# yoseph007/PQA2

Measured on AMD Instinct MI355X. Metric: VMAF frames/sec (vif+adm+motion2 -> SVM), device-resident synthetic YUV pairs, higher is better.
Workload: dtype f32; 1 GPU; 2160p 3840x2160 8-bit, vmaf_4k_v0.6.1, 300 frames/GPU; frames_per_gpu=300, frames_total=300, batch=97, frames_per_launch=75, clips_pipelined=True, parallelism=frame-shard x1, 1-frame motion halo, all-gather of records + of scores

## Files before the change

include/pqa_vmaf.h:

```cpp
#ifndef PQA_VMAF_H
#define PQA_VMAF_H

#include <stddef.h>
#include <stdint.h>

#if defined(__GNUC__)
#define PQA_API __attribute__((visibility("default")))
#else
#define PQA_API
#endif

#ifdef __cplusplus
extern "C" {
#endif

typedef enum pqa_status {
  PQA_OK = 0,
  PQA_EINVAL = -1,
  PQA_EDEVICE = -2,
  PQA_ENOMEM = -3,
  PQA_ECANCELLED = -4,
  PQA_ESTATE = -5
} pqa_status;

// ... 335 lines not shown
  uint32_t width, height;
} pqa_edge_spec;
PQA_API int pqa_edge_profiles(pqa_ctx* ctx, const pqa_edge_spec* spec, const void* const* ref_frames, int64_t ref_row_stride,
                              const void* const* dis_frames, int64_t dis_row_stride, int32_t n_frames, uint64_t* out);
PQA_API int pqa_edge_profiles_device(pqa_ctx* ctx, const pqa_edge_spec* spec, const void* ref, int64_t ref_row_pitch,
                                     int64_t ref_frame_pitch, const void* dis, int64_t dis_row_pitch, int64_t dis_frame_pitch,
                                     int32_t n_frames, uint64_t* out);
PQA_API int pqa_edge_sums(void);

PQA_API int pqa_colour_sums(void);
PQA_API int pqa_colour_moments_device(pqa_ctx* ctx, const pqa_device_clip* ref, const pqa_device_clip* dis, int32_t n_frames,
                                      uint32_t lo, uint32_t hi, uint64_t* out);
PQA_API int pqa_colour_moments(pqa_ctx* ctx, const void* const* ref_frames, const int64_t ref_strides[3],
                               const void* const* dis_frames, const int64_t dis_strides[3], int32_t n_frames, uint32_t lo,
                               uint32_t hi, uint64_t* out);

PQA_API int pqa_colour_apply_device(pqa_ctx* ctx, const int32_t m[12], const pqa_device_clip* src, const pqa_device_clip* dst,
                                    int32_t n_frames);
PQA_API int pqa_colour_apply(pqa_ctx* ctx, const int32_t m[12], const void* const* src_frames, const int64_t src_strides[3],
                             void* const* dst_frames, const int64_t dst_strides[3], int32_t n_frames);

enum { PQA_GRAY_LUMA = 0, PQA_GRAY_BT601_FULL = 1 };
PQA_API int pqa_set_luma_gray(pqa_ctx* ctx, uint32_t mode);

enum { PQA_PROF_KERNELS = 17 };
PQA_API int pqa_profile_enable(pqa_ctx* ctx, int on);
PQA_API int pqa_profile_read(pqa_ctx* ctx, int kernel_id, double* total_ms, uint64_t* launches, uint64_t* frames);
PQA_API const char* pqa_profile_kernel_name(int kernel_id);

PQA_API int pqa_debug_vif_march_table(uint16_t* out, int32_t capacity_halfwords);

PQA_API int pqa_debug_vif_march_shape(uint32_t width, uint32_t height, int32_t* out6);

PQA_API int pqa_debug_ciede2000(const double* lab_pairs, int32_t n, double* de_out);

enum { PQA_CAMBI_PARAM_INTS = 22 };
PQA_API int pqa_debug_cambi_params(uint32_t w, uint32_t h, uint32_t bit_depth, int32_t* out, int32_t cap);

PQA_API int pqa_debug_cambi_cmap(const void* luma, int64_t row_pitch_bytes, uint32_t w, uint32_t h, uint32_t bit_depth,
                                 float* cmap, int64_t cap, double* score);

PQA_API int pqa_debug_psnr_hvs_dct8x8(const int32_t* in, int32_t* out, int32_t n);

enum { PQA_PSNR_HVS_TABLE_FLOATS = 384 };
PQA_API int pqa_debug_psnr_hvs_tables(float* out, int32_t cap);

PQA_API int pqa_debug_psnr_hvs_plane(const void* ref, const void* dis, int64_t row_pitch_bytes, uint32_t w, uint32_t h,
                                     uint32_t bit_depth, uint32_t plane_kind, float* block_err, double* mse);

PQA_API int pqa_debug_xpsnr_blocks(const void* ref, const void* ref_m1, const void* ref_m2, const void* dis,
                                   int64_t row_pitch_bytes, uint32_t w, uint32_t h, uint32_t bit_depth, int32_t hfr,
                                   uint64_t* out, double* wsse);

PQA_API int pqa_debug_siti_plane(const void* cur, const void* prev, int64_t row_pitch_bytes, uint32_t w, uint32_t h,
                                 uint32_t bit_depth, int32_t full_range, float* gmap, double* si_ti);

PQA_API int pqa_debug_resample_table(uint32_t filter, int32_t n_src, int32_t n_dst, int64_t x0_q16, int64_t ext_q16,
                                     int32_t* first, int16_t* coeff, int32_t cap_taps, int32_t* taps);

PQA_API int pqa_debug_colour(uint32_t bit_depth, uint32_t hshift, uint32_t vshift, uint32_t w, uint32_t h,
                             const void* const ref[3], const void* const dis[3], uint32_t lo, uint32_t hi, uint64_t* sums28,
                             const int32_t* m, void* const applied[3]);

#ifdef __cplusplus
}
#endif
// ... 2 lines not shown
```

pqa2_amd/_native.py:

```python
from __future__ import annotations

import ctypes as C
import os
import subprocess

_HERE = os.path.dirname(os.path.abspath(__file__))
LIB_PATH = os.environ.get("PQA_LIB_PATH") or os.path.join(_HERE, "csrc", "libpqa_vmaf.so")

PQA_OK, PQA_EINVAL, PQA_EDEVICE, PQA_ENOMEM, PQA_ECANCELLED, PQA_ESTATE = 0, -1, -2, -3, -4, -5
FEAT_VIF, FEAT_ADM, FEAT_MOTION, FEAT_PSNR, FEAT_SSIM = 1, 2, 4, 8, 16
FEAT_VMAF = FEAT_VIF | FEAT_ADM | FEAT_MOTION
FEAT_ALL = FEAT_VMAF | FEAT_PSNR | FEAT_SSIM
FEAT_FLOAT_SSIM, FEAT_MS_SSIM = 32, 64
FEAT_CIEDE = 256
FEAT_CAMBI, FEAT_CAMBI_FULL_REF = 512, 1024
FEAT_PSNR_HVS = 2048
FEAT_XPSNR, FEAT_XPSNR_HFR = 4096, 8192
FEAT_SITI, FEAT_SITI_REF_FULL, FEAT_SITI_DIS_FULL = 16384, 32768, 65536
FEAT_INTEGRITY = 131072
FEAT_KNOWN = (FEAT_ALL | FEAT_FLOAT_SSIM | FEAT_MS_SSIM | FEAT_CIEDE | FEAT_CAMBI | FEAT_CAMBI_FULL_REF | FEAT_PSNR_HVS
              | FEAT_XPSNR | FEAT_XPSNR_HFR | FEAT_SITI | FEAT_SITI_REF_FULL | FEAT_SITI_DIS_FULL
              | FEAT_INTEGRITY)
VIF_BORDER_FLOAT, VIF_BORDER_INTEGER = 0, 1
FIXED_VIF, FIXED_MOTION, FIXED_ADM, FIXED_ALL = 1, 2, 4, 7
REC_VIF_NUM, REC_VIF_DEN, REC_ADM_NUM, REC_ADM_DEN, REC_MOTION, REC_SSIM, REC_SSE = 0, 4, 8, 12, 16, 17, 20
RECORD_DOUBLES = 24
EXT_FLOAT_SSIM, EXT_FLOAT_SSIM_LCS, EXT_MS_SSIM, EXT_MS_SSIM_L, EXT_MS_SSIM_C, EXT_MS_SSIM_S, EXT_RESERVED = 0, 1, 4, 5, 10, 15, 20
EXT_CIEDE2000, EXT_CIEDE_MEAN_DE = 20, 21
EXT_CAMBI, EXT_CAMBI_SOURCE = 22, 23
CAMBI_PARAM_INTS = 22
EXT_DOUBLES = 24
EXT2_PSNR_HVS_Y, EXT2_PSNR_HVS_CB, EXT2_PSNR_HVS_CR, EXT2_PSNR_HVS, EXT2_PSNR_HVS_MSE, EXT2_RESERVED = 0, 1, 2, 3, 4, 7
EXT2_DOUBLES = 8
EXT3_XPSNR_Y, EXT3_XPSNR_U, EXT3_XPSNR_V, EXT3_WSSE, EXT3_RESERVED = 0, 1, 2, 3, 6
EXT3_DOUBLES = 8
EXT4_SI, EXT4_TI, EXT4_SI_SOURCE, EXT4_TI_SOURCE, EXT4_RESERVED = 0, 1, 2, 3, 4
EXT4_DOUBLES = 8
EXT5_SAD_PREV, EXT5_BLACK_COUNT, EXT5_RESERVED = 0, 3, 4
EXT5_DOUBLES = 8
PSNR_HVS_TABLE_FLOATS = 384
PROF_KERNELS = 17
GRAY_LUMA, GRAY_BT601_FULL = 0, 1

EXPORTS = [
    "pqa_version", "pqa_record_doubles", "pqa_ext_doubles", "pqa_ext2_doubles", "pqa_ext3_doubles", "pqa_ext4_doubles", "pqa_ext5_doubles", "pqa_config_init", "pqa_create", "pqa_destroy", "pqa_set_stream",
    "pqa_submit", "pqa_submit_fd", "pqa_submit_fd_run", "pqa_submit_device", "pqa_submit_surfaces", "pqa_submit_packed", "pqa_set_motion_halo", "pqa_set_ref_history", "pqa_set_dis_history", "pqa_set_dis_history_planes", "pqa_set_black_threshold", "pqa_frame_sad", "pqa_frame_sad_device", "pqa_flush", "pqa_collect", "pqa_collect_ext", "pqa_collect_ext2", "pqa_collect_ext3", "pqa_collect_ext4", "pqa_collect_ext5", "pqa_sync",
    "pqa_cancel", "pqa_reset", "pqa_last_error", "pqa_luma_stats_device", "pqa_luma_stats", "pqa_cross_sse_device", "pqa_cross_sse", "pqa_shift_sse_device", "pqa_shift_sse", "pqa_level_stats_device", "pqa_level_stats", "pqa_level_bins", "pqa_resample", "pqa_resample_device", "pqa_unpack", "pqa_unpack_device", "pqa_format_convert", "pqa_format_convert_device", "pqa_flow_moments", "pqa_flow_moments_device", "pqa_line_profiles", "pqa_line_profiles_device", "pqa_tile_moments", "pqa_tile_moments_device", "pqa_band_moments", "pqa_band_moments_device", "pqa_band_sums", "pqa_temporal_moments", "pqa_temporal_moments_device", "pqa_temporal_sums", "pqa_edge_profiles", "pqa_edge_profiles_device", "pqa_edge_sums", "pqa_colour_sums", "pqa_colour_moments", "pqa_colour_moments_device", "pqa_colour_apply", "pqa_colour_apply_device", "pqa_set_luma_gray",
    "pqa_profile_enable",
    "pqa_profile_read", "pqa_profile_kernel_name", "pqa_debug_vif_march_table", "pqa_debug_vif_march_shape",
    "pqa_debug_ciede2000", "pqa_debug_cambi_params", "pqa_debug_cambi_cmap", "pqa_debug_psnr_hvs_dct8x8",
    "pqa_debug_psnr_hvs_tables", "pqa_debug_psnr_hvs_plane", "pqa_debug_xpsnr_blocks", "pqa_debug_siti_plane",
    "pqa_debug_resample_table", "pqa_debug_colour",
]


class PqaConfig(C.Structure):
    _fields_ = [
        ("struct_size", C.c_uint32), ("device", C.c_int32), ("width", C.c_uint32), ("height", C.c_uint32),
        ("bit_depth", C.c_uint32), ("n_planes", C.c_uint32), ("chroma_hshift", C.c_uint32),
        ("chroma_vshift", C.c_uint32), ("features", C.c_uint32), ("max_batch", C.c_uint32),
        ("result_capacity", C.c_uint32), ("n_subsample", C.c_uint32),
        ("vif_enhn_gain_limit", C.c_double), ("adm_enhn_gain_limit", C.c_double),
        ("vif_border", C.c_uint32), ("fixed_point", C.c_uint32),
    ]


class PqaDeviceClip(C.Structure):
    _fields_ = [("plane", C.c_void_p * 3), ("row_pitch", C.c_int64 * 3), ("frame_pitch", C.c_int64 * 3)]


SURFACE_NV12, SURFACE_P01X = 1, 2
SURFACE_PLANAR, SURFACE_UYVY, SURFACE_YUYV, SURFACE_V210 = 0, 3, 4, 5
PACKED_FORMATS = {"uyvy422": SURFACE_UYVY, "yuyv422": SURFACE_YUYV, "v210": SURFACE_V210}
PACKED_BIT_DEPTH = {SURFACE_UYVY: 8, SURFACE_YUYV: 8, SURFACE_V210: 10}


class PqaSurfaceClip(C.Structure):
    _fields_ = [("struct_size", C.c_uint32), ("format", C.c_uint32), ("luma", C.c_void_p), ("chroma", C.c_void_p),
                ("luma_row_pitch", C.c_int64), ("luma_frame_pitch", C.c_int64),
                ("chroma_row_pitch", C.c_int64), ("chroma_frame_pitch", C.c_int64)]


# ... 173 lines not shown
    lib.pqa_line_profiles.argtypes = [vp, C.POINTER(PqaProfileSpec), C.POINTER(vp), i64, i32, vp]
    lib.pqa_line_profiles_device.argtypes = [vp, C.POINTER(PqaProfileSpec), vp, i64, i64, i32, vp]
    lib.pqa_tile_moments.argtypes = [vp, C.POINTER(PqaTileSpec), C.POINTER(vp), i64, C.POINTER(vp), i64, i32, vp]
    lib.pqa_tile_moments_device.argtypes = [vp, C.POINTER(PqaTileSpec), vp, i64, i64, vp, i64, i64, i32, vp]
    lib.pqa_band_moments.argtypes = [vp, C.POINTER(PqaBandSpec), C.POINTER(vp), i64, C.POINTER(vp), i64, i32, vp]
    lib.pqa_band_moments_device.argtypes = [vp, C.POINTER(PqaBandSpec), vp, i64, i64, vp, i64, i64, i32, vp]
    lib.pqa_temporal_moments.argtypes = [vp, C.POINTER(PqaTemporalSpec), C.POINTER(vp), i64, C.POINTER(vp), i64, i32, vp]
    lib.pqa_temporal_moments_device.argtypes = [vp, C.POINTER(PqaTemporalSpec), vp, i64, i64, vp, i64, i64, i32, vp]
    lib.pqa_temporal_sums.argtypes = []
    lib.pqa_temporal_sums.restype = C.c_int
    lib.pqa_edge_profiles.argtypes = [vp, C.POINTER(PqaEdgeSpec), C.POINTER(vp), i64, C.POINTER(vp), i64, i32, vp]
    lib.pqa_edge_profiles_device.argtypes = [vp, C.POINTER(PqaEdgeSpec), vp, i64, i64, vp, i64, i64, i32, vp]
    lib.pqa_edge_sums.argtypes = []
    lib.pqa_edge_sums.restype = C.c_int
    lib.pqa_band_sums.argtypes = []
    lib.pqa_band_sums.restype = C.c_int
    lib.pqa_colour_sums.argtypes = []
    lib.pqa_colour_sums.restype = C.c_int
    lib.pqa_colour_moments_device.argtypes = [vp, C.POINTER(PqaDeviceClip), C.POINTER(PqaDeviceClip), i32, C.c_uint32, C.c_uint32, vp]
    lib.pqa_colour_moments.argtypes = [vp, C.POINTER(vp), C.POINTER(i64 * 3), C.POINTER(vp), C.POINTER(i64 * 3), i32, C.c_uint32, C.c_uint32, vp]
    lib.pqa_colour_apply_device.argtypes = [vp, C.POINTER(i32 * 12), C.POINTER(PqaDeviceClip), C.POINTER(PqaDeviceClip), i32]
    lib.pqa_colour_apply.argtypes = [vp, C.POINTER(i32 * 12), C.POINTER(vp), C.POINTER(i64 * 3), C.POINTER(vp), C.POINTER(i64 * 3), i32]
    lib.pqa_debug_colour.argtypes = [C.c_uint32, C.c_uint32, C.c_uint32, C.c_uint32, C.c_uint32, C.POINTER(vp * 3), C.POINTER(vp * 3),
                                     C.c_uint32, C.c_uint32, vp, C.POINTER(i32 * 12), C.POINTER(vp * 3)]
    lib.pqa_debug_resample_table.argtypes = [C.c_uint32, i32, i32, i64, i64, vp, vp, i32, C.POINTER(i32)]
    lib.pqa_set_luma_gray.argtypes = [vp, C.c_uint32]
    lib.pqa_reset.argtypes = [vp]
    lib.pqa_last_error.argtypes = [vp]
    lib.pqa_last_error.restype = C.c_char_p
    lib.pqa_profile_enable.argtypes = [vp, C.c_int]
    lib.pqa_profile_read.argtypes = [vp, C.c_int, C.POINTER(dbl), C.POINTER(C.c_uint64), C.POINTER(C.c_uint64)]
    lib.pqa_debug_vif_march_table.argtypes = [vp, i32]
    lib.pqa_debug_vif_march_shape.argtypes = [C.c_uint32, C.c_uint32, C.POINTER(i32 * 6)]
    lib.pqa_debug_ciede2000.argtypes = [vp, i32, vp]
    lib.pqa_debug_cambi_params.argtypes = [C.c_uint32, C.c_uint32, C.c_uint32, vp, i32]
    lib.pqa_debug_cambi_cmap.argtypes = [vp, C.c_int64, C.c_uint32, C.c_uint32, C.c_uint32, vp, C.c_int64, vp]
    lib.pqa_debug_psnr_hvs_dct8x8.argtypes = [vp, vp, i32]
    lib.pqa_debug_psnr_hvs_tables.argtypes = [vp, i32]
    lib.pqa_debug_psnr_hvs_plane.argtypes = [vp, vp, C.c_int64, C.c_uint32, C.c_uint32, C.c_uint32, C.c_uint32, vp, vp]
    lib.pqa_debug_xpsnr_blocks.argtypes = [vp, vp, vp, vp, C.c_int64, C.c_uint32, C.c_uint32, C.c_uint32, i32, vp, vp]
    lib.pqa_debug_siti_plane.argtypes = [vp, vp, C.c_int64, C.c_uint32, C.c_uint32, C.c_uint32, i32, vp, vp]
    lib.pqa_profile_kernel_name.argtypes = [C.c_int]
    lib.pqa_profile_kernel_name.restype = C.c_char_p
    assert lib.pqa_record_doubles() == RECORD_DOUBLES
    assert lib.pqa_ext_doubles() == EXT_DOUBLES
    assert lib.pqa_ext2_doubles() == EXT2_DOUBLES
    assert lib.pqa_ext3_doubles() == EXT3_DOUBLES
    assert lib.pqa_ext4_doubles() == EXT4_DOUBLES
    assert lib.pqa_ext5_doubles() == EXT5_DOUBLES
    assert lib.pqa_colour_sums() == COLOUR_SUMS
    _lib = lib
    return lib
```

pqa2_amd/csrc/kernels.h:

```cpp
#pragma once
#include <hip/hip_runtime.h>
#include <stdint.h>

#include <vector>

namespace pqa {

enum Elem : int { ELEM_U8 = 0, ELEM_U16 = 1, ELEM_F32 = 2 };

struct PlaneRun {
  const void* base;
  int64_t row_pitch;
  int64_t frame_pitch;
};

struct MutPlaneRun {
  void* base;
  int64_t row_pitch;
  int64_t frame_pitch;
};

int vif_tile_w(int scale);
constexpr int kVifTileH = 8;
inline int vif_tiles_x(int scale, int w) { return (w + vif_tile_w(scale) - 1) / vif_tile_w(scale); }
inline int vif_tiles_y(int h) { return (h + kVifTileH - 1) / kVifTileH; }

enum : int { VIF_S0_VALU = 0, VIF_S0_AUTO = 1 };
hipError_t launch_vif_stat(hipStream_t stream, int scale, Elem elem, PlaneRun ref, PlaneRun dis, int n_frames,
                           int w, int h, float inv_scale, float gain_limit, int border101, double* partials,
                           MutPlaneRun next_ref, MutPlaneRun next_dis, int s0_mode = VIF_S0_AUTO, int* n_partials = nullptr,
                           int uniform = 1);
hipError_t vif_march_prepare();
int vif_march_partials_max(int w, int h);
int vif_march_table(uint16_t* out, int capacity_halfwords);
void vif_march_shape(int w, int h, int* out6);
bool launch_vif_s0_march(hipStream_t stream, Elem elem, int bits, PlaneRun ref, PlaneRun dis, int n_frames, int w, int h, float gain_limit,
                         int border101, double* partials, MutPlaneRun next_ref, MutPlaneRun next_dis, int* n_partials,
                         hipError_t* err, int uniform = 1);
constexpr int kVifFxPartials = 8;
void vif_fixed_log2_table(uint16_t* out32768);
hipError_t launch_vif_fixed(hipStream_t stream, int scale, int bit_depth, Elem elem, PlaneRun ref, PlaneRun dis,
                            int n_frames, int w, int h, double gain_limit, const uint16_t* log2_lut,
                            long long* partials, MutPlaneRun next_ref, MutPlaneRun next_dis);

constexpr int kAdmTileW = 60, kAdmTileH = 14;
inline int adm_tiles_x(int band_w) { return (band_w + kAdmTileW - 1) / kAdmTileW; }
inline int adm_tiles_y(int band_h) { return (band_h + kAdmTileH - 1) / kAdmTileH; }

enum : int { ADM_TILED = 0, ADM_AUTO = 1, ADM_MARCH = 2 };
hipError_t launch_adm_scale(hipStream_t stream, int scale, Elem elem, PlaneRun ref, PlaneRun dis, int n_frames,
                            int w, int h, float inv_scale, float gain_limit, MutPlaneRun ll_ref,
                            MutPlaneRun ll_dis, double* partials, int mode = ADM_AUTO, int* n_partials = nullptr);
int adm_march_partials(int band_w, int band_h);
bool launch_adm_march(hipStream_t stream, int scale, Elem elem, PlaneRun ref, PlaneRun dis, int n_frames, int w, int h,
                      float inv_scale, float gain_limit, MutPlaneRun ll_ref, MutPlaneRun ll_dis, double* partials,
                      int* n_partials, hipError_t* err);
bool adm_pyramid_takes(Elem elem, int w, int h);
int adm_pyramid_partials(int w, int h);
bool launch_adm_pyramid(hipStream_t stream, Elem elem, PlaneRun ref, PlaneRun dis, int n_frames, int w, int h, float inv_scale,
                        float gain_limit, MutPlaneRun ll_ref, MutPlaneRun ll_dis, double* partials0, double* partials1,
                        int* n_partials, hipError_t* err);
float adm_dwt_quant_step(int lambda, int theta);

constexpr int kAdmFxRows = kAdmTileH + 2;
// ... 320 lines not shown
```

pqa2_amd/csrc/pqa_api.hip:

```cpp
#include "pqa_ctx.h"

#include <algorithm>
#include <cstdarg>
#include <cstdio>
#include <cstdlib>
#include <mutex>

#include "ingest.h"

using namespace pqa;
using pqa::host::PackPool;
using pqa::host::PackTask;
using pqa::host::run_pack_task;

static thread_local std::string g_create_error;

int pqa::fail(pqa_ctx* c, int code, const char* fmt, ...) {
  char buf[512];
  va_list ap;
  va_start(ap, fmt);
  vsnprintf(buf, sizeof buf, fmt, ap);
  va_end(ap);
  if (c) c->err = buf; else g_create_error = buf;
  return code;
// ... 142 lines not shown
struct Scale { int s; Elem elem; RunPair in; int w, h; MutRunPair out; };

template <typename Launch>
int walk_pyramid(const Level (&lv)[4], Scale first, Elem deep, Launch launch) {
  for (Scale k = first; k.s < 4; ++k.s) {
    k.out = k.s < 3 ? level_out(lv[k.s + 1]) : MutRunPair{};
    const int rc = launch(k);
    if (rc != PQA_OK) return rc;
    if (k.s < 3) {
      const Level& L = lv[k.s + 1];
      k.in = level_in(L);
      k.elem = deep;
      k.w = L.w; k.h = L.h;
    }
  }
  return PQA_OK;
}

int run_vif(pqa_ctx* c, Batch& b) {
  if (!(c->cfg.features & PQA_FEAT_VIF) || b.sp_n == 0) return PQA_OK;
  const Scale top{0, c->elem, RunPair{b.rs[0], b.ds[0]}, b.w, b.h, {}};
  if (c->vif_fixed)
    return walk_pyramid(c->vif_lv, top, ELEM_U16, [&](const Scale& k) -> int {
      ProfScope ps(c, k.s, b.sp_n, b.st);
      HIPCHK(c, launch_vif_fixed(b.st, k.s, (int)c->cfg.bit_depth, k.elem, k.in.ref, k.in.dis, b.sp_n, k.w, k.h,
                                 c->cfg.vif_enhn_gain_limit, c->vif_lut, c->vif_fx_part[k.s], k.out.ref, k.out.dis));
      return PQA_OK;
    });
  return walk_pyramid(c->vif_lv, top, ELEM_F32, [&](const Scale& k) -> int {
    {
      ProfScope ps(c, k.s, b.sp_n, b.st);
      HIPCHK(c, launch_vif_stat(b.st, k.s, k.elem, k.in.ref, k.in.dis, b.sp_n, k.w, k.h, c->inv_scale,
                                (float)c->cfg.vif_enhn_gain_limit, c->cfg.vif_border == PQA_VIF_BORDER_INTEGER, c->vif_part[k.s],
                                k.out.ref, k.out.dis, c->vif_s0_mode, &b.vif_np[k.s], c->vif_uniform));
    }
    return k.s == 0 && b.fork_late ? fork_streams(c, b) : PQA_OK;
  });
}

int run_adm(pqa_ctx* c, Batch& b) {
  if (!(c->cfg.features & PQA_FEAT_ADM) || b.sp_n == 0) return PQA_OK;
  Scale top{0, c->elem, RunPair{b.rs[0], b.ds[0]}, b.w, b.h, {}};
  if (c->adm_fixed)
    return walk_pyramid(c->adm_lv, top, ELEM_F32, [&](const Scale& k) -> int {
      ProfScope ps(c, 7 + k.s, b.sp_n, b.st_adm);
      HIPCHK(c, launch_adm_fixed(b.st_adm, k.s, (int)c->cfg.bit_depth, k.elem, k.in.ref, k.in.dis, b.sp_n, k.w, k.h,
                                 c->cfg.adm_enhn_gain_limit, c->adm_div_lut, k.out.ref, k.out.dis, c->adm_fx_part[k.s]));
      return PQA_OK;
    });
  if (c->adm_mode == ADM_AUTO) {
    const Level& L2 = c->adm_lv[2];
    hipError_t perr = hipSuccess;
    int np = 0;
    ProfScope ps(c, 7, b.sp_n, b.st_adm);
    if (launch_adm_pyramid(b.st_adm, top.elem, top.in.ref, top.in.dis, b.sp_n, top.w, top.h, c->inv_scale,
                           (float)c->cfg.adm_enhn_gain_limit, level_out(L2).ref, level_out(L2).dis, c->adm_part[0], c->adm_part[1],
                           &np, &perr)) {
      HIPCHK(c, perr);
      b.adm_np[0] = b.adm_np[1] = np;
      top = Scale{2, ELEM_F32, level_in(L2), L2.w, L2.h, {}};
    }
  }
  return walk_pyramid(c->adm_lv, top, ELEM_F32, [&](const Scale& k) -> int {
    ProfScope ps(c, 7 + k.s, b.sp_n, b.st_adm);
    HIPCHK(c, launch_adm_scale(b.st_adm, k.s, k.elem, k.in.ref, k.in.dis, b.sp_n, k.w, k.h, c->inv_scale,
                               (float)c->cfg.adm_enhn_gain_limit, k.out.ref, k.out.dis, c->adm_part[k.s], c->adm_mode, &b.adm_np[k.s]));
    return PQA_OK;
// ... 667 lines not shown
  if (c->cfg.adm_enhn_gain_limit <= 0) c->cfg.adm_enhn_gain_limit = 100.0;
  c->elem = cfg->bit_depth > 8 ? ELEM_U16 : ELEM_U8;
  c->esize = cfg->bit_depth > 8 ? 2 : 1;
  c->inv_scale = 1.0f / (float)(1 << (cfg->bit_depth - 8));
  c->n_planes = (int)cfg->n_planes;
  c->pw[0] = (int)cfg->width; c->ph[0] = (int)cfg->height;
  for (int p = 1; p < 3; ++p) {
    c->pw[p] = (int)((cfg->width + (1u << cfg->chroma_hshift) - 1) >> cfg->chroma_hshift);
    c->ph[p] = (int)((cfg->height + (1u << cfg->chroma_vshift) - 1) >> cfg->chroma_vshift);
  }

  auto bail = [&](int rc) {
    g_create_error = c->err;
    pqa_destroy(c);
    return rc;
  };
#define CREATE_TRY(expr) do { int rc_ = (expr); if (rc_ != PQA_OK) return bail(rc_); } while (0)
#define CREATE_HIP(expr) do { hipError_t e_ = (expr); if (e_ != hipSuccess) { \
    fail(c, e_ == hipErrorOutOfMemory ? PQA_ENOMEM : PQA_EDEVICE, "%s failed: %s", #expr, hipGetErrorString(e_)); \
    return bail(e_ == hipErrorOutOfMemory ? PQA_ENOMEM : PQA_EDEVICE); } } while (0)

  CREATE_HIP(hipSetDevice(c->device));
  CREATE_HIP(hipStreamCreateWithFlags(&c->own_stream, hipStreamNonBlocking));
  c->stream = c->own_stream;
  {
    const char* e = getenv("PQA_MULTI_STREAM");
    c->multi_stream = (e && e[0] == '1') ? 1 : (e && e[0] == '2') ? 2 : 0;
    const char* t = getenv("PQA_TRACE");
    c->trace = t && t[0] == '1';
    const char* v = getenv("PQA_VIF_MFMA");
    c->vif_s0_mode = (v && v[0] == '0') ? VIF_S0_VALU : VIF_S0_AUTO;
    const char* vu = getenv("PQA_VIF_UNIFORM");
    c->vif_uniform = !(vu && vu[0] == '0');
    const char* am = getenv("PQA_ADM_MARCH");
    const char* ap = getenv("PQA_ADM_PYRAMID");
    c->adm_mode = (am && am[0] == '0') ? ADM_TILED : (ap && ap[0] == '0') ? ADM_MARCH : ADM_AUTO;
    const char* mm = getenv("PQA_MOTION_MARCH");
    c->motion_mode = (mm && mm[0] == '0') ? MOTION_TILED : MOTION_AUTO;
    const char* xm = getenv("PQA_XSSE_MFMA");
    c->xsse_mfma = !(xm && xm[0] == '0');
    const char* tw = getenv("PQA_TEMPORAL_WALK");
    c->temporal_walk = tw && tw[0] == '1';
  }
  for (int i = 0; i < 2; ++i) {
    CREATE_HIP(hipStreamCreateWithFlags(&c->aux[i], hipStreamNonBlocking));
    CREATE_HIP(hipEventCreateWithFlags(&c->join_ev[i], hipEventDisableTiming));
  }
  CREATE_HIP(hipEventCreateWithFlags(&c->fork_ev, hipEventDisableTiming));
  for (int i = 0; i < kBatchEvents; ++i) CREATE_HIP(hipEventCreateWithFlags(&c->batch_ev[i], hipEventDisableTiming));
  try {
    c->ring.init(c->capacity);
  } catch (...) {
    fail(c, PQA_ENOMEM, "out of host memory");
    return bail(PQA_ENOMEM);
  }

  c->vif_fixed = (cfg->features & PQA_FEAT_VIF) && (cfg->fixed_point & PQA_FIXED_VIF);
  c->motion_fixed = (cfg->features & PQA_FEAT_MOTION) && (cfg->fixed_point & PQA_FIXED_MOTION);
  c->adm_fixed = (cfg->features & PQA_FEAT_ADM) && (cfg->fixed_point & PQA_FIXED_ADM);
  if (c->adm_fixed) {
    std::vector<int32_t> lut(65537);
    adm_fixed_div_table(lut.data());
    CREATE_TRY(dev_alloc(c, &c->adm_div_lut, lut.size()));
    CREATE_HIP(hipMemcpy(c->adm_div_lut, lut.data(), lut.size() * sizeof(int32_t), hipMemcpyHostToDevice));
  }
  if ((cfg->features & PQA_FEAT_VIF) && !c->vif_fixed) CREATE_HIP(vif_march_prepare());
// ... 919 lines not shown
```

pqa2_amd/csrc/pqa_ctx.h:

```cpp
#pragma once
#include "../../include/pqa_vmaf.h"

#include <atomic>
#include <cstring>
#include <memory>
#include <string>
#include <thread>
#include <vector>

#include "host_chain.h"
#include "host_pack.h"
#include "host_ring.h"
#include "host_packed.h"
#include "host_stage.h"
#include "kernels.h"

namespace pqa {

struct Level {
  int w = 0, h = 0;
  int64_t pitch = 0, frame_pitch = 0;
  float* ref = nullptr;
  float* dis = nullptr;
};
// ... 137 lines not shown
  pqa::HistPlane mo_hist;
  pqa::host::FrameChain mo_chain;
  pqa::Half half[2];
  int cur_half = 0, pending = 0;
  int64_t pending_first = 0;
  size_t slot_bytes = 0;
  size_t plane_off[2][3] = {};
  int64_t slot_row_pitch[3] = {};
  bool staging_ready = false;
  std::thread pin_thread;
  hipError_t pin_err = hipSuccess;
  uint8_t* surf_dev = nullptr;
  uint8_t* pk_pin[2][2] = {};
  uint8_t* pk_dev[2][2] = {};
  size_t pk_pin_cap[2][2] = {}, pk_dev_cap[2][2] = {};
  hipStream_t pk_stream = nullptr;
  hipEvent_t pk_copied[2] = {nullptr, nullptr}, pk_computed[2] = {nullptr, nullptr};
  bool pk_copied_pending[2] = {false, false}, pk_computed_pending[2] = {false, false};
  int pk_set = 0;
  std::unique_ptr<pqa::host::PackPool> pack_pool;
  bool pack_pool_tried = false;
  std::vector<pqa::host::PackTask> pack_tasks;
  pqa::host::RecordRing ring;
  hipEvent_t batch_ev[pqa::kBatchEvents] = {};
  uint64_t batch_ev_seq[pqa::kBatchEvents] = {};
  uint64_t batch_seq = 0;
  uint64_t done_seq = 0;
  std::atomic<int> cancelled{0};
  std::string err;
  std::vector<void*> allocs;
  int multi_stream = 0;
  int vif_s0_mode = pqa::VIF_S0_AUTO;
  int vif_uniform = 1;
  int adm_mode = pqa::ADM_AUTO;
  int motion_mode = pqa::MOTION_AUTO;
  bool trace = false;
  bool prof = false;
  uint32_t prof_mask = 0xffffffffu;
  std::vector<pqa::ProfEv> evs;
  double prof_ms[PQA_PROF_KERNELS] = {};
  uint64_t prof_n[PQA_PROF_KERNELS] = {}, prof_frames[PQA_PROF_KERNELS] = {};
};

namespace pqa {

int fail(pqa_ctx* c, int code, const char* fmt, ...);

#define HIPCHK(c, expr)                                                                          \
  do {                                                                                           \
    hipError_t e_ = (expr);                                                                      \
    if (e_ != hipSuccess)                                                                        \
      return pqa::fail((c), e_ == hipErrorOutOfMemory ? PQA_ENOMEM : PQA_EDEVICE, "%s failed: %s", #expr, \
                  hipGetErrorString(e_));                                                        \
  } while (0)

template <typename T>
int dev_alloc(pqa_ctx* c, T** out, size_t count) {
  void* p = nullptr;
  if (count == 0) count = 1;
  HIPCHK(c, hipMalloc(&p, count * sizeof(T)));
  c->allocs.push_back(p);
  *out = (T*)p;
  return PQA_OK;
}

}
// ... 1 lines not shown
```

pqa2_amd/csrc/pqa_debug.hip:

```cpp
#include "pqa_ctx.h"

using namespace pqa;

namespace {

int need_device() {
  int ndev = 0;
  if (hipGetDeviceCount(&ndev) != hipSuccess || ndev <= 0)
    return fail(nullptr, PQA_EDEVICE, "no HIP device visible (this library has no CPU fallback)");
  return PQA_OK;
}

int plane_pitch_rule(const char* who, uint32_t bit_depth, uint32_t w, int64_t row_pitch_bytes, int* es) {
  *es = bit_depth > 8 ? 2 : 1;
  if (row_pitch_bytes < (int64_t)w * *es || row_pitch_bytes % *es)
    return fail(nullptr, PQA_EINVAL, "%s: bad row pitch %lld", who, (long long)row_pitch_bytes);
  return PQA_OK;
}

struct Scratch {
  void* held[12];
  int n = 0;
  hipError_t err = hipSuccess;
  ~Scratch() { for (int i = 0; i < n; ++i) hipFree(held[i]); }
  template <typename T>
  T* get(size_t count) {
    void* p = nullptr;
    if (err == hipSuccess) err = n < 12 ? hipMalloc(&p, count * sizeof(T)) : hipErrorOutOfMemory;
    if (p) held[n++] = p;
    return (T*)p;
  }
  void* plane(const void* host, int64_t row_pitch_bytes, size_t row_bytes, uint32_t h) {
    if (!host) return nullptr;
    void* p = get<uint8_t>(row_bytes * h);
    if (err == hipSuccess) err = hipMemcpy2D(p, row_bytes, host, (size_t)row_pitch_bytes, row_bytes, h, hipMemcpyHostToDevice);
    return p;
  }
};

}

extern "C" {

int pqa_debug_vif_march_table(uint16_t* out, int32_t capacity_halfwords) { return vif_march_table(out, capacity_halfwords); }
int pqa_debug_vif_march_shape(uint32_t width, uint32_t height, int32_t* out6) {
  if (!out6 || width == 0 || height == 0 || width > 65536 || height > 65536) return PQA_EINVAL;
  int shape[6];
  vif_march_shape((int)width, (int)height, shape);
  for (int i = 0; i < 6; ++i) out6[i] = shape[i];
  return PQA_OK;
}

int pqa_debug_ciede2000(const double* lab_pairs, int32_t n, double* de_out) {
  if (n < 0 || (n > 0 && (!lab_pairs || !de_out))) return fail(nullptr, PQA_EINVAL, "bad argument");
  const int rc = need_device();
  if (rc != PQA_OK) return rc;
  if (n == 0) return PQA_OK;
  std::vector<float> in((size_t)n * 6), out((size_t)n);
  for (size_t i = 0; i < in.size(); ++i) in[i] = (float)lab_pairs[i];
  Scratch s;
  float* d_in = s.get<float>(in.size());
  float* d_out = s.get<float>(out.size());
  hipError_t e = s.err;
  if (e == hipSuccess) e = hipMemcpy(d_in, in.data(), in.size() * sizeof(float), hipMemcpyHostToDevice);
  if (e == hipSuccess) e = launch_ciede_debug(nullptr, d_in, n, d_out);
  if (e == hipSuccess) e = hipMemcpy(out.data(), d_out, out.size() * sizeof(float), hipMemcpyDeviceToHost);
  if (e != hipSuccess) return fail(nullptr, PQA_EDEVICE, "pqa_debug_ciede2000: %s", hipGetErrorString(e));
  for (int32_t i = 0; i < n; ++i) de_out[i] = (double)out[i];
  return PQA_OK;
}

int pqa_debug_cambi_params(uint32_t w, uint32_t h, uint32_t bit_depth, int32_t* out, int32_t cap) {
  if (!out || cap < PQA_CAMBI_PARAM_INTS) return fail(nullptr, PQA_EINVAL, "pqa_debug_cambi_params: null or short output");
  if (w < 16 || h < 16 || w > 16384 || h > 16384 || (bit_depth != 8 && bit_depth != 10))
    return fail(nullptr, PQA_EINVAL, "pqa_debug_cambi_params: unsupported %ux%u at %u bit", w, h, bit_depth);
  static_assert(kCambiParamInts == PQA_CAMBI_PARAM_INTS, "pqa_debug_cambi_params layout");
  const CambiParams p = cambi_params((int)w, (int)h);
  int i = 0;
  out[i++] = p.ws; out[i++] = p.r; out[i++] = p.piw; out[i++] = p.mask_t;
  for (int d = 0; d < kCambiDiffs; ++d) out[i++] = p.tvi[d];
  for (int d = 0; d < kCambiDiffs; ++d) out[i++] = p.weights[d];
  for (int s = 0; s < kCambiScales; ++s) { out[i++] = p.sw[s]; out[i++] = p.sh[s]; }
// ... 238 lines not shown
```

pqa2_amd/csrc/vif.hip:

```cpp
#include <cstring>
#include <mutex>
#include <vector>

#include <cstdio>
#include "kernels.h"
#include "pqa_device.h"

namespace pqa {

namespace {

struct Taps {
  float f[17];
};

static Taps gaussian_taps(int n) {
  Taps t{};
  double v[17], sum = 0.0;
  const double sigma = n / 5.0;
  for (int k = 0; k < n; ++k) {
    const double d = k - n / 2;
    v[k] = exp(-0.5 * d * d / (sigma * sigma));
    sum += v[k];
  }
// ... 251 lines not shown
              }
            }
#pragma unroll
            for (int p = 0; p < S / 2; ++p) {
              const int k = j - 2 * p;
              if (k >= 0 && k <= N) {
                const f2 c = a.taps.vt[k];
                acc[p][0] = __builtin_elementwise_fma(c, f2{r, r}, acc[p][0]);
                acc[p][1] = __builtin_elementwise_fma(c, f2{d, d}, acc[p][1]);
                acc[p][2] = __builtin_elementwise_fma(c, f2{rr, rr}, acc[p][2]);
                acc[p][3] = __builtin_elementwise_fma(c, f2{dd, dd}, acc[p][3]);
                acc[p][4] = __builtin_elementwise_fma(c, f2{rd, rd}, acc[p][4]);
              }
            }
          }
        }
        __builtin_amdgcn_sched_barrier(0);
      }
#pragma unroll
      for (int p = 0; p < S / 2; ++p)
#pragma unroll
        for (int s = 0; s < 5; ++s) sv[s][seg * (S / 2) + p][col] = acc[p][s];
      if (ND) {
#pragma unroll
        for (int q = 0; q < S / 2; ++q) sd[seg * (S / 2) + q][col] = dacc[q];
      }
    }
  }
  __syncthreads();

  vif_hstat<N, TW, ND>(a, &sv[0][0][0], &sd[0][0], red, fr, tile, x0, y0);
}


template <int N, int TW, int ND>
hipError_t launch_stat_n(hipStream_t stream, Elem elem, const VifStatArgs& a, int n_frames) {
  const dim3 grid(a.n_tiles, n_frames), block(kBlock);
  switch (elem) {
    case ELEM_U8: hipLaunchKernelGGL((vif_stat_kernel<uint8_t, N, TW, ND>), grid, block, 0, stream, a); break;
    case ELEM_U16: hipLaunchKernelGGL((vif_stat_kernel<uint16_t, N, TW, ND>), grid, block, 0, stream, a); break;
    case ELEM_F32: hipLaunchKernelGGL((vif_stat_kernel<float, N, TW, ND>), grid, block, 0, stream, a); break;
  }
  return hipGetLastError();
}

constexpr int kVifN[4] = {17, 9, 5, 3};
constexpr int kVifTW[4] = {240, 248, 252, 252};

}

int vif_tile_w(int scale) { return kVifTW[scale]; }

hipError_t launch_vif_stat(hipStream_t stream, int scale, Elem elem, PlaneRun ref, PlaneRun dis, int n_frames,
                           int w, int h, float inv_scale, float gain_limit, int border101, double* partials,
                           MutPlaneRun next_ref, MutPlaneRun next_dis, int s0_mode, int* n_partials, int uniform) {
  if (n_partials) *n_partials = vif_tiles_x(scale, w) * vif_tiles_y(h);
  if (n_frames <= 0) return hipSuccess;
  const int bits = elem == ELEM_U8 ? 8 : (elem == ELEM_U16 && inv_scale == 0.25f) ? 10 : (elem == ELEM_U16 && inv_scale == 0.0625f) ? 12 : 0;
  if (scale == 0 && bits && s0_mode == VIF_S0_AUTO && next_ref.base && next_dis.base) {
    hipError_t err = hipSuccess;
    if (launch_vif_s0_march(stream, elem, bits, ref, dis, n_frames, w, h, gain_limit, border101, partials, next_ref, next_dis, n_partials, &err, uniform))
      return err;
    if (n_partials) *n_partials = vif_tiles_x(scale, w) * vif_tiles_y(h);
  }
  VifStatArgs a{};
  a.ref = ref.base; a.dis = dis.base;
  a.row_pitch_r = ref.row_pitch; a.frame_pitch_r = ref.frame_pitch;
  a.row_pitch_d = dis.row_pitch; a.frame_pitch_d = dis.frame_pitch;
  a.w = w; a.h = h;
  a.fold_w = 2 * w - (border101 ? 2 : 1); a.fold_h = 2 * h - (border101 ? 2 : 1);
  a.tiles_x = vif_tiles_x(scale, w);
  a.n_tiles = a.tiles_x * vif_tiles_y(h);
  a.inv_scale = inv_scale; a.gain_limit = gain_limit;
  a.uniform = uniform;
  a.partials = partials;
  a.dst_ref = (float*)next_ref.base; a.dst_dis = (float*)next_dis.base;
  a.dst_row_pitch_r = next_ref.row_pitch; a.dst_frame_pitch_r = next_ref.frame_pitch;
  a.dst_row_pitch_d = next_dis.row_pitch; a.dst_frame_pitch_d = next_dis.frame_pitch;
  const Taps cur = gaussian_taps(kVifN[scale]);
  const Taps nxt = scale < 3 ? gaussian_taps(kVifN[scale + 1]) : Taps{};
  a.taps = tap_pairs(cur, kVifN[scale], scale < 3 ? &nxt : nullptr, scale < 3 ? kVifN[scale + 1] : 0);
  if (scale < 3 && (!a.dst_ref || !a.dst_dis)) return hipErrorInvalidValue;
  switch (scale) {
    case 0: return launch_stat_n<17, 240, 9>(stream, elem, a, n_frames);
    case 1: return launch_stat_n<9, 248, 5>(stream, elem, a, n_frames);
    case 2: return launch_stat_n<5, 252, 3>(stream, elem, a, n_frames);
    case 3: return launch_stat_n<3, 252, 0>(stream, elem, a, n_frames);
  }
  return hipErrorInvalidValue;
}

}
```

Before: 22980 frames/s.

## Add VIF strip kernel that carries vertical filter accumulators across tile rows

Adds a strip-marching VIF statistic kernel for scales 1-3 on float input. Each workgroup walks a vertical segment of tiles and keeps the partial vertical-filter sums in registers for the tile below, so the halo rows are not re-read and re-filtered per tile. Loads for the next tile row are issued before the current row is stored and reduced. It is enabled by default only for scale 1 (mask 0x2), with the segment length chosen automatically from occupancy heuristics. The trade is fewer workgroups and more register pressure, against less redundant halo traffic.

```diff
diff --git a/include/pqa_vmaf.h b/include/pqa_vmaf.h
--- a/include/pqa_vmaf.h
+++ b/include/pqa_vmaf.h
@@ -391,6 +391,8 @@
 
 PQA_API int pqa_debug_vif_march_shape(uint32_t width, uint32_t height, int32_t* out6);
 
+PQA_API int pqa_debug_vif_strip_shape(pqa_ctx* ctx, uint32_t scale, uint32_t n_frames, int32_t* out4);
+
 PQA_API int pqa_debug_ciede2000(const double* lab_pairs, int32_t n, double* de_out);
 
 enum { PQA_CAMBI_PARAM_INTS = 22 };
diff --git a/pqa2_amd/_native.py b/pqa2_amd/_native.py
--- a/pqa2_amd/_native.py
+++ b/pqa2_amd/_native.py
@@ -47,7 +47,7 @@
     "pqa_submit", "pqa_submit_fd", "pqa_submit_fd_run", "pqa_submit_device", "pqa_submit_surfaces", "pqa_submit_packed", "pqa_set_motion_halo", "pqa_set_ref_history", "pqa_set_dis_history", "pqa_set_dis_history_planes", "pqa_set_black_threshold", "pqa_frame_sad", "pqa_frame_sad_device", "pqa_flush", "pqa_collect", "pqa_collect_ext", "pqa_collect_ext2", "pqa_collect_ext3", "pqa_collect_ext4", "pqa_collect_ext5", "pqa_sync",
     "pqa_cancel", "pqa_reset", "pqa_last_error", "pqa_luma_stats_device", "pqa_luma_stats", "pqa_cross_sse_device", "pqa_cross_sse", "pqa_shift_sse_device", "pqa_shift_sse", "pqa_level_stats_device", "pqa_level_stats", "pqa_level_bins", "pqa_resample", "pqa_resample_device", "pqa_unpack", "pqa_unpack_device", "pqa_format_convert", "pqa_format_convert_device", "pqa_flow_moments", "pqa_flow_moments_device", "pqa_line_profiles", "pqa_line_profiles_device", "pqa_tile_moments", "pqa_tile_moments_device", "pqa_band_moments", "pqa_band_moments_device", "pqa_band_sums", "pqa_temporal_moments", "pqa_temporal_moments_device", "pqa_temporal_sums", "pqa_edge_profiles", "pqa_edge_profiles_device", "pqa_edge_sums", "pqa_colour_sums", "pqa_colour_moments", "pqa_colour_moments_device", "pqa_colour_apply", "pqa_colour_apply_device", "pqa_set_luma_gray",
     "pqa_profile_enable",
-    "pqa_profile_read", "pqa_profile_kernel_name", "pqa_debug_vif_march_table", "pqa_debug_vif_march_shape",
+    "pqa_profile_read", "pqa_profile_kernel_name", "pqa_debug_vif_march_table", "pqa_debug_vif_march_shape", "pqa_debug_vif_strip_shape",
     "pqa_debug_ciede2000", "pqa_debug_cambi_params", "pqa_debug_cambi_cmap", "pqa_debug_psnr_hvs_dct8x8",
     "pqa_debug_psnr_hvs_tables", "pqa_debug_psnr_hvs_plane", "pqa_debug_xpsnr_blocks", "pqa_debug_siti_plane",
     "pqa_debug_resample_table", "pqa_debug_colour",
@@ -287,6 +287,7 @@
     lib.pqa_profile_read.argtypes = [vp, C.c_int, C.POINTER(dbl), C.POINTER(C.c_uint64), C.POINTER(C.c_uint64)]
     lib.pqa_debug_vif_march_table.argtypes = [vp, i32]
     lib.pqa_debug_vif_march_shape.argtypes = [C.c_uint32, C.c_uint32, C.POINTER(i32 * 6)]
+    lib.pqa_debug_vif_strip_shape.argtypes = [vp, C.c_uint32, C.c_uint32, C.POINTER(i32 * 4)]
     lib.pqa_debug_ciede2000.argtypes = [vp, i32, vp]
     lib.pqa_debug_cambi_params.argtypes = [C.c_uint32, C.c_uint32, C.c_uint32, vp, i32]
     lib.pqa_debug_cambi_cmap.argtypes = [vp, C.c_int64, C.c_uint32, C.c_uint32, C.c_uint32, vp, C.c_int64, vp]
diff --git a/pqa2_amd/csrc/kernels.h b/pqa2_amd/csrc/kernels.h
--- a/pqa2_amd/csrc/kernels.h
+++ b/pqa2_amd/csrc/kernels.h
@@ -29,7 +29,8 @@
 hipError_t launch_vif_stat(hipStream_t stream, int scale, Elem elem, PlaneRun ref, PlaneRun dis, int n_frames,
                            int w, int h, float inv_scale, float gain_limit, int border101, double* partials,
                            MutPlaneRun next_ref, MutPlaneRun next_dis, int s0_mode = VIF_S0_AUTO, int* n_partials = nullptr,
-                           int uniform = 1);
+                           int uniform = 1, int strip_seg = 0);
+void vif_strip_shape(int scale, int w, int h, int n_frames, int strip_seg, int* out4);
 hipError_t vif_march_prepare();
 int vif_march_partials_max(int w, int h);
 int vif_march_table(uint16_t* out, int capacity_halfwords);
diff --git a/pqa2_amd/csrc/pqa_api.hip b/pqa2_amd/csrc/pqa_api.hip
--- a/pqa2_amd/csrc/pqa_api.hip
+++ b/pqa2_amd/csrc/pqa_api.hip
@@ -198,7 +198,8 @@
       ProfScope ps(c, k.s, b.sp_n, b.st);
       HIPCHK(c, launch_vif_stat(b.st, k.s, k.elem, k.in.ref, k.in.dis, b.sp_n, k.w, k.h, c->inv_scale,
                                 (float)c->cfg.vif_enhn_gain_limit, c->cfg.vif_border == PQA_VIF_BORDER_INTEGER, c->vif_part[k.s],
-                                k.out.ref, k.out.dis, c->vif_s0_mode, &b.vif_np[k.s], c->vif_uniform));
+                                k.out.ref, k.out.dis, c->vif_s0_mode, &b.vif_np[k.s], c->vif_uniform,
+                                (c->vif_strip_mask >> k.s & 1) ? c->vif_strip_seg : -1));
     }
     return k.s == 0 && b.fork_late ? fork_streams(c, b) : PQA_OK;
   });
@@ -932,6 +933,10 @@
     c->vif_s0_mode = (v && v[0] == '0') ? VIF_S0_VALU : VIF_S0_AUTO;
     const char* vu = getenv("PQA_VIF_UNIFORM");
     c->vif_uniform = !(vu && vu[0] == '0');
+    const char* vs = getenv("PQA_VIF_STRIP");
+    if (vs && vs[0]) c->vif_strip_mask = atoi(vs) & 0xe;
+    const char* vg = getenv("PQA_VIF_STRIP_SEG");
+    c->vif_strip_seg = vg ? std::max(0, atoi(vg)) : 0;
     const char* am = getenv("PQA_ADM_MARCH");
     const char* ap = getenv("PQA_ADM_PYRAMID");
     c->adm_mode = (am && am[0] == '0') ? ADM_TILED : (ap && ap[0] == '0') ? ADM_MARCH : ADM_AUTO;
diff --git a/pqa2_amd/csrc/pqa_ctx.h b/pqa2_amd/csrc/pqa_ctx.h
--- a/pqa2_amd/csrc/pqa_ctx.h
+++ b/pqa2_amd/csrc/pqa_ctx.h
@@ -193,6 +193,8 @@
   int multi_stream = 0;
   int vif_s0_mode = pqa::VIF_S0_AUTO;
   int vif_uniform = 1;
+  int vif_strip_mask = 0x2;
+  int vif_strip_seg = 0;
   int adm_mode = pqa::ADM_AUTO;
   int motion_mode = pqa::MOTION_AUTO;
   bool trace = false;
diff --git a/pqa2_amd/csrc/pqa_debug.hip b/pqa2_amd/csrc/pqa_debug.hip
--- a/pqa2_amd/csrc/pqa_debug.hip
+++ b/pqa2_amd/csrc/pqa_debug.hip
@@ -48,6 +48,18 @@
   int shape[6];
   vif_march_shape((int)width, (int)height, shape);
   for (int i = 0; i < 6; ++i) out6[i] = shape[i];
+  return PQA_OK;
+}
+
+int pqa_debug_vif_strip_shape(pqa_ctx* ctx, uint32_t scale, uint32_t n_frames, int32_t* out4) {
+  if (!ctx) return PQA_EINVAL;
+  if (!out4 || scale < 1 || scale > 3 || n_frames == 0 || n_frames > 65536)
+    return fail(ctx, PQA_EINVAL, "pqa_debug_vif_strip_shape: bad argument");
+  const Level& L = ctx->vif_lv[scale];
+  int shape[4];
+  const int strip_seg = ctx->vif_fixed ? -1 : (ctx->vif_strip_mask >> scale & 1) ? ctx->vif_strip_seg : -1;
+  vif_strip_shape((int)scale, L.w, L.h, (int)n_frames, strip_seg, shape);
+  for (int i = 0; i < 4; ++i) out4[i] = shape[i];
   return PQA_OK;
 }
 
diff --git a/pqa2_amd/csrc/vif.hip b/pqa2_amd/csrc/vif.hip
--- a/pqa2_amd/csrc/vif.hip
+++ b/pqa2_amd/csrc/vif.hip
@@ -307,6 +307,168 @@
   vif_hstat<N, TW, ND>(a, &sv[0][0][0], &sd[0][0], red, fr, tile, x0, y0);
 }
 
+template <int N, int ND>
+__device__ __forceinline__ void vif_strip_row(const TapPairs& taps, const int j, f2 x , f2 (&cur)[4][5],
+                                              f2 (&cd)[4], f2 (&nxt)[4][5], f2 (&nd)[4]) {
+  constexpr int R = N / 2, RD = ND / 2, S = kVifTileH;
+  asm volatile("" : "+v"(x));
+  const f2 xx = x * x;
+  const float r = x.x, d = x.y, rr = xx.x, dd = xx.y, rd = x.x * x.y;
+  if (ND) {
+#pragma unroll
+    for (int q = 0; q < S / 2; ++q) {
+      const int kd = j - (2 * q + R - RD);
+      if (kd >= 0 && kd < ND) cd[q] = __builtin_elementwise_fma(taps.dt[kd], x, cd[q]);
+      if (kd - S >= 0 && kd - S < ND) nd[q] = __builtin_elementwise_fma(taps.dt[kd - S], x, nd[q]);
+    }
+  }
+#pragma unroll
+  for (int p = 0; p < S / 2; ++p) {
+    const int k = j - 2 * p;
+    if (k >= 0 && k <= N) {
+      const f2 c = taps.vt[k];
+      cur[p][0] = __builtin_elementwise_fma(c, f2{r, r}, cur[p][0]);
+      cur[p][1] = __builtin_elementwise_fma(c, f2{d, d}, cur[p][1]);
+      cur[p][2] = __builtin_elementwise_fma(c, f2{rr, rr}, cur[p][2]);
+      cur[p][3] = __builtin_elementwise_fma(c, f2{dd, dd}, cur[p][3]);
+      cur[p][4] = __builtin_elementwise_fma(c, f2{rd, rd}, cur[p][4]);
+    }
+    if (k - S >= 0 && k - S <= N) {
+      const f2 c = taps.vt[k - S];
+      nxt[p][0] = __builtin_elementwise_fma(c, f2{r, r}, nxt[p][0]);
+      nxt[p][1] = __builtin_elementwise_fma(c, f2{d, d}, nxt[p][1]);
+      nxt[p][2] = __builtin_elementwise_fma(c, f2{rr, rr}, nxt[p][2]);
+      nxt[p][3] = __builtin_elementwise_fma(c, f2{dd, dd}, nxt[p][3]);
+      nxt[p][4] = __builtin_elementwise_fma(c, f2{rd, rd}, nxt[p][4]);
+    }
+  }
+}
+
+template <int N, int ND>
+__device__ __forceinline__ void vif_strip_rows(const TapPairs& taps, const f2 (&xc)[8], f2 (&cur)[4][5], f2 (&cd)[4],
+                                               f2 (&nxt)[4][5], f2 (&nd)[4]) {
+  constexpr int NRP = kVifTileH / 2;
+#pragma unroll
+  for (int p = 0; p < NRP; ++p) {
+#pragma unroll
+    for (int s = 0; s < 5; ++s) nxt[p][s] = f2{0.0f, 0.0f};
+    nd[p] = f2{0.0f, 0.0f};
+  }
+#pragma unroll
+  for (int i = 0; i < 8; ++i) {
+    vif_strip_row<N, ND>(taps, N - 1 + i, xc[i], cur, cd, nxt, nd);
+    if (i & 1) __builtin_amdgcn_sched_barrier(0);
+  }
+}
+
+template <int ND>
+__device__ __forceinline__ void vif_strip_store(const f2 (&cur)[4][5], const f2 (&cd)[4], f2* sv, f2* sd, const int col) {
+  constexpr int NRP = kVifTileH / 2;
+#pragma unroll
+  for (int p = 0; p < NRP; ++p)
+#pragma unroll
+    for (int s = 0; s < 5; ++s) sv[(s * NRP + p) * kP2 + col] = cur[p][s];
+  if (ND) {
+#pragma unroll
+    for (int q = 0; q < NRP; ++q) sd[q * kP2 + col] = cd[q];
+  }
+}
+
+__device__ __forceinline__ const VifStatArgs& vif_strip_kernargs() {
+  auto p = __builtin_amdgcn_kernarg_segment_ptr();
+  asm volatile("" : "+s"(p));
+  return *(const VifStatArgs*)p;
+}
+
+template <int N, int TW, int ND>
+__global__ __launch_bounds__(kBlock, 3) void vif_strip_kernel(const VifStatArgs a, const int tiles_y, const int seg_len,
+                                                              const int n_segs) {
+  constexpr int R = N / 2, TH = kVifTileH, COLS = TW + N - 1, NSEG = TW / 4, S = 8;
+  static_assert(ND == 0 || ND / 2 <= R, "decimation window must sit inside the statistic window");
+  static_assert(COLS <= 256 && COLS <= kP2, "one column per thread");
+  static_assert(TW % 4 == 0 && NSEG <= 64 && TH == S, "segment map");
+  static_assert(N - 1 <= S, "the prologue fits one load group; a row feeds at most the tile below");
+  __shared__ f2 sv[5][TH / 2][kP2];
+  __shared__ f2 sd[ND ? TH / 2 : 1][ND ? kP2 : 1];
+  __shared__ double red[12];
+
+  const int wg = xcd_remap(blockIdx.x, a.tiles_x * n_segs);
+  const int tx = wg % a.tiles_x, sg = wg / a.tiles_x;
+  const int fr = blockIdx.y;
+  const int ty0 = sg * seg_len, ty1 = min(ty0 + seg_len, tiles_y);
+  const float* __restrict__ ref = (const float*)a.ref + (int64_t)fr * a.frame_pitch_r;
+  const float* __restrict__ dis = (const float*)a.dis + (int64_t)fr * a.frame_pitch_d;
+  const int x0 = tx * TW;
+  const int col = threadIdx.x;
+
+  const unsigned gx = (unsigned)mirror_fold(x0 - R + col, a.w, a.fold_w);
+  const unsigned pitch_r = (unsigned)a.row_pitch_r, pitch_d = (unsigned)a.row_pitch_d;
+  const auto rsrc_r = make_rsrc(ref, (unsigned)a.h * pitch_r * (unsigned)sizeof(float));
+  const auto rsrc_d = make_rsrc(dis, (unsigned)a.h * pitch_d * (unsigned)sizeof(float));
+
+  f2 accA[S / 2][5], accB[S / 2][5], dA[S / 2], dB[S / 2];
+  f2 xn[S];
+  auto issue = [&](const int y0, const bool more) __attribute__((always_inline)) {
+    const int ylo = y0 + R;
+    const unsigned gxs = more ? gx : 0x3fffffffu;
+    unsigned ro_r[S], ro_d[S];
+    unsigned sp_r = pitch_r, sp_d = pitch_d;
+    asm volatile("" : "+s"(sp_r), "+s"(sp_d));
+#pragma unroll
+    for (int i = 0; i < S; ++i) {
+      const unsigned gy = (unsigned)mirror_fold(ylo + i, a.h, a.fold_h);
+      ro_r[i] = gy * sp_r; ro_d[i] = gy * sp_d;
+    }
+#pragma unroll
+    for (int i = 0; i < S; ++i) {
+      xn[i].x = buf_load<float>(rsrc_r, gxs, ro_r[i]);
+      xn[i].y = buf_load<float>(rsrc_d, gxs, ro_d[i]);
+      __builtin_amdgcn_sched_barrier(0);
+    }
+  };
+
+  {
+    f2 px[N - 1];
+#pragma unroll
+    for (int j = 0; j < N - 1; ++j) {
+      const unsigned gy = (unsigned)mirror_fold(ty0 * TH - R + j, a.h, a.fold_h);
+      px[j].x = buf_load<float>(rsrc_r, gx, gy * pitch_r);
+      px[j].y = buf_load<float>(rsrc_d, gx, gy * pitch_d);
+    }
+    issue(ty0 * TH, true);
+#pragma unroll
+    for (int p = 0; p < S / 2; ++p) {
+#pragma unroll
+      for (int s = 0; s < 5; ++s) accA[p][s] = accB[p][s] = f2{0.0f, 0.0f};
+      dA[p] = dB[p] = f2{0.0f, 0.0f};
+    }
+#pragma unroll
+    for (int j = 0; j < N - 1; ++j) vif_strip_row<N, ND>(a.taps, j, px[j], accA, dA, accB, dB);
+  }
+
+  auto step = [&](const int ty, f2 (&cur)[S / 2][5], f2 (&cd)[S / 2], f2 (&nxt)[S / 2][5], f2 (&nd)[S / 2]) __attribute__((always_inline)) {
+    vif_strip_rows<N, ND>(vif_strip_kernargs().taps, xn, cur, cd, nxt, nd);
+    issue((ty + 1) * TH, ty + 1 < ty1);
+    __syncthreads();
+    vif_strip_store<ND>(cur, cd, &sv[0][0][0], &sd[0][0], col);
+    __syncthreads();
+    int x0s = x0, frs = fr;
+    asm volatile("" : "+s"(x0s), "+s"(frs));
+    vif_hstat<N, TW, ND>(vif_strip_kernargs(), &sv[0][0][0], &sd[0][0], red, frs, ty * a.tiles_x + tx, x0s, ty * TH);
+  };
+  for (int ty = ty0; ty < ty1; ty += 2) {
+    step(ty, accA, dA, accB, dB);
+    if (ty + 1 >= ty1) break;
+    step(ty + 1, accB, dB, accA, dA);
+  }
+}
+
+template <int N, int TW, int ND>
+hipError_t launch_strip_n(hipStream_t stream, const VifStatArgs& a, int n_frames, const int (&shape)[4]) {
+  const dim3 grid(shape[0] * shape[3], n_frames), block(kBlock);
+  hipLaunchKernelGGL((vif_strip_kernel<N, TW, ND>), grid, block, 0, stream, a, shape[1], shape[2], shape[3]);
+  return hipGetLastError();
+}
 
 template <int N, int TW, int ND>
 hipError_t launch_stat_n(hipStream_t stream, Elem elem, const VifStatArgs& a, int n_frames) {
@@ -326,9 +488,27 @@
 
 int vif_tile_w(int scale) { return kVifTW[scale]; }
 
+void vif_strip_shape(int scale, int w, int h, int n_frames, int strip_seg, int* out) {
+  const int strips = vif_tiles_x(scale, w), tiles_y = vif_tiles_y(h);
+  int seg = 0;
+  if (scale >= 1 && scale <= 3 && strip_seg > 0) {
+    seg = strip_seg < tiles_y ? strip_seg : tiles_y;
+  } else if (scale >= 1 && scale <= 3 && strip_seg == 0) {
+    constexpr int kSegRows = 9;
+    const double round = 3.0 * 256;
+    for (int s = tiles_y < kSegRows ? tiles_y : kSegRows; s >= 2 && !seg; --s) {
+      const int n = (tiles_y + s - 1) / s;
+      if ((tiles_y + n - 1) / n != s) continue;
+      if ((double)strips * n * n_frames >= 8.0 * round) seg = s;
+    }
+  }
+  const int n_segs = seg ? (tiles_y + seg - 1) / seg : 0;
+  out[0] = strips; out[1] = tiles_y; out[2] = seg; out[3] = n_segs;
+}
+
 hipError_t launch_vif_stat(hipStream_t stream, int scale, Elem elem, PlaneRun ref, PlaneRun dis, int n_frames,
                            int w, int h, float inv_scale, float gain_limit, int border101, double* partials,
-                           MutPlaneRun next_ref, MutPlaneRun next_dis, int s0_mode, int* n_partials, int uniform) {
+                           MutPlaneRun next_ref, MutPlaneRun next_dis, int s0_mode, int* n_partials, int uniform, int strip_seg) {
   if (n_partials) *n_partials = vif_tiles_x(scale, w) * vif_tiles_y(h);
   if (n_frames <= 0) return hipSuccess;
   const int bits = elem == ELEM_U8 ? 8 : (elem == ELEM_U16 && inv_scale == 0.25f) ? 10 : (elem == ELEM_U16 && inv_scale == 0.0625f) ? 12 : 0;
@@ -356,6 +536,15 @@
   const Taps nxt = scale < 3 ? gaussian_taps(kVifN[scale + 1]) : Taps{};
   a.taps = tap_pairs(cur, kVifN[scale], scale < 3 ? &nxt : nullptr, scale < 3 ? kVifN[scale + 1] : 0);
   if (scale < 3 && (!a.dst_ref || !a.dst_dis)) return hipErrorInvalidValue;
+  if (elem == ELEM_F32 && scale >= 1) {
+    int shape[4];
+    vif_strip_shape(scale, w, h, n_frames, strip_seg, shape);
+    if (shape[2]) switch (scale) {
+      case 1: return launch_strip_n<9, 248, 5>(stream, a, n_frames, shape);
+      case 2: return launch_strip_n<5, 252, 3>(stream, a, n_frames, shape);
+      case 3: return launch_strip_n<3, 252, 0>(stream, a, n_frames, shape);
+    }
+  }
   switch (scale) {
     case 0: return launch_stat_n<17, 240, 9>(stream, elem, a, n_frames);
     case 1: return launch_stat_n<9, 248, 5>(stream, elem, a, n_frames);
```

Result: faster. 23240 frames/s (median of 6 runs) (+1.1%).
